# thiagopbueno/tf-mpc

Hardware: AMD Instinct MI355X
Metric: iLQR iterations/sec (batch x horizon) at n=16,m=8,T=50 (higher is better)
Workload: dtype f32

## Files before the change

tf-mpc_amd/csrc/lqr_mfma16x8.hip:

```cpp
#include <hip/hip_runtime.h>

#include <cstdlib>
#include <cstring>
#include <type_traits>

#include "lqr_kernels.h"
#include "options.h"
#include "mfma_bf16x3.h"
#include "wave_ldlt8.h"
#include "wave_ldlt8_pair.h"
#include "wave_ops.h"

namespace tfmpc {

namespace {

constexpr int N = 16, M = 8, D = 24;
using f32x4 = bf3::f32x4;

__device__ __forceinline__ f32x4 mfma(float a, float b, f32x4 c)
{
    return __builtin_amdgcn_mfma_f32_16x16x4f32(a, b, c, 0, 0, 0);
}

__device__ __forceinline__ float readlane(float v, int lane)
{
    return __builtin_bit_cast(float, __builtin_amdgcn_readlane(__builtin_bit_cast(int, v), lane));
}

using namespace bf3;

constexpr int kMs = 0;
constexpr int kKs = 256;
constexpr int kVt = 512;
constexpr int kVtLd = 20;
constexpr int kSweepFloats = kVt + 16 * kVtLd;
constexpr int kZs = 0;
constexpr int kZld = 26;
#ifndef TFMPC_LQR_TC
#define TFMPC_LQR_TC 52
#endif
constexpr int kTC = TFMPC_LQR_TC;
constexpr int kRolloutFloats = kZs + (kTC + 1) * kZld + 6;
constexpr int kLdsFloats = kSweepFloats > kRolloutFloats ? kSweepFloats : kRolloutFloats;
static_assert(kLdsFloats % 4 == 0, "slices are 16-byte aligned (pair_src, the 16-byte accesses of the sweep)");
#ifndef TFMPC_LQR_RING
#define TFMPC_LQR_RING 4
#endif
constexpr int kRing = TFMPC_LQR_RING;
static_assert(kTC % kRing == 0, "a chunk must hold whole turns of the gain ring");

template <int CTRL>
__device__ __forceinline__ float dpp(float v)
{
    return __builtin_bit_cast(float, __builtin_amdgcn_update_dpp(0, __builtin_bit_cast(int, v), CTRL, 0xF, 0xF, false));
}
constexpr int kDppXor1 = 0xB1;
constexpr int kDppXor2 = 0x4E;
constexpr int kDppHalfMirror = 0x141;

#define TFMPC_GLOBAL __attribute__((address_space(1)))
using gbytes = TFMPC_GLOBAL char *;
__device__ __forceinline__ gbytes uniform_base(const float *p)
{
    gbytes g = (gbytes)p;
    asm("" : "+s"(g));
    return g;
}
__device__ __forceinline__ unsigned here(unsigned &off)
{
    asm volatile("" : "+v"(off));
    return off;
}
template <class V>
__device__ __forceinline__ V gload(gbytes base, unsigned &off) { return *reinterpret_cast<const TFMPC_GLOBAL V *>(base + here(off)); }
template <class V>
__device__ __forceinline__ void gstore(gbytes base, unsigned &off, V v) { *reinterpret_cast<TFMPC_GLOBAL V *>(base + here(off)) = v; }
__device__ __forceinline__ int pinned(int v)
{
    asm("" : "+v"(v));
    return v;
}
typedef float f32x4_lds __attribute__((ext_vector_type(4), aligned(8)));
typedef float f32x4_any __attribute__((ext_vector_type(4), aligned(4)));

#ifdef TFMPC_LQR_EU
#define TFMPC_LQR_WAVES(EU_) TFMPC_LQR_EU
#else
#define TFMPC_LQR_WAVES(EU_) (EU_)
#endif
#define TFMPC_LQR_OCCUPANCY __attribute__((amdgpu_waves_per_eu(TFMPC_LQR_WAVES(EU), TFMPC_LQR_WAVES(EU))))
__device__ __forceinline__ void block_lds_sync()
{
    __builtin_amdgcn_fence(__ATOMIC_RELEASE, "workgroup", "local");
    __builtin_amdgcn_s_barrier();
    __builtin_amdgcn_fence(__ATOMIC_ACQUIRE, "workgroup", "local");
}
template <bool BACKWARD, bool FORWARD, bool VALUE, bool EXACT, bool BF3, bool OUT16 = false, int EU = 4, bool PAIR = false>
__global__ __launch_bounds__(PAIR ? 2 * kWave : kWave) TFMPC_LQR_OCCUPANCY void lqr_mfma16x8_kernel(LqrArgs a)
{
    static_assert(!PAIR || (BACKWARD && !VALUE && !OUT16), "the paired elimination serves the sweeps without value outputs");
    __shared__ __attribute__((aligned(16))) float lds_all[(PAIR ? 2 : 1) * kLdsFloats];
    const int wave = PAIR ? __builtin_amdgcn_readfirstlane(threadIdx.x >> 6) : 0;
    float *const lds = lds_all + wave * kLdsFloats;
    const int b_own = PAIR ? 2 * (int)blockIdx.x + wave : (int)blockIdx.x;
    const bool live = !PAIR || b_own < a.B;
    const int b = live ? b_own : a.B - 1;
    const int lane = PAIR ? (int)(threadIdx.x & (kWave - 1)) : (int)threadIdx.x;
    const int i = lane & 15, q = lane >> 4;
    const int T = a.T;
    const int n = EXACT ? N : a.n, m = EXACT ? M : a.m, d = n + m;
    auto Fxx = [&](const float *Fg, int row, int xi) { return (row < n && xi < n) ? Fg[row * d + xi] : 0.0f; };
    auto Fxu = [&](const float *Fg, int row, int ui) { return (row < n && ui < m) ? Fg[row * d + n + ui] : 0.0f; };
    auto zmap = [&](int zi) { return zi < N ? (zi < n ? zi : -1) : (zi - N < m ? n + zi - N : -1); };
    auto Czz = [&](const float *Cg, int zr, int zc) {
        const int r = zmap(zr), c_ = zmap(zc);
        return (r >= 0 && c_ >= 0) ? Cg[r * d + c_] : 0.0f;
    };
    auto cz = [&](const float *cg, int zr) { const int r = zmap(zr); return r >= 0 ? cg[r] : 0.0f; };
    const float *Fg = a.F + (size_t)b * a.sF;
    const float *fg = a.f + (size_t)b * a.sf;
    const float *Cg = a.C + (size_t)b * a.sC;
    const float *cg = a.c + (size_t)b * a.sc;
    float *Kg = a.K + (size_t)b * a.sK;
    float *kg = a.k + (size_t)b * a.sk;
    int status = 0;

    if (BACKWARD) {
        float Fb0[4], Fb1[4];
        f32x4 Cd00, Cd11;
        f32x4 Cd01t;
        f32x4 vterm;
#pragma unroll
        for (int r = 0; r < 4; ++r) {
            const int k = 4 * q + r;
            const int ku = N + k;
            if (EXACT) {
                Fb0[r] = Fg[k * D + i];
                Fb1[r] = (i < M) ? Fg[k * D + N + i] : ((i == M) ? fg[k] : 0.0f);
                Cd00[r] = Cg[k * D + i];
                Cd01t[r] = (k < M) ? Cg[(N + k) * D + i] : ((k == M) ? cg[i] : 0.0f);
                vterm[r] = (i == M) ? cg[k] : 0.0f;
                Cd11[r] = (ku < D) ? ((i < M) ? Cg[ku * D + N + i] : ((i == M) ? cg[ku] : 0.0f)) : 0.0f;
            } else {
                Fb0[r] = Fxx(Fg, k, i);
                Fb1[r] = (i < M) ? Fxu(Fg, k, i) : ((i == M && k < n) ? fg[k] : 0.0f);
                Cd00[r] = Czz(Cg, k, i);
                Cd01t[r] = (k < M) ? Czz(Cg, N + k, i) : ((k == M) ? cz(cg, i) : 0.0f);
                vterm[r] = (i == M) ? cz(cg, k) : 0.0f;
                float c11 = 0.0f;
                if (ku < D) {
                    if (i < M) c11 = (k >= m && i == k) ? 1.0f : Czz(Cg, ku, N + i);
                    else if (i == M) c11 = cz(cg, ku);
                }
                Cd11[r] = c11;
            }
        }
        ConstFrag Fc0{}, Fc1{};
        if (BF3) {
            Fc0 = const_frag(f32x4{Fb0[0], Fb0[1], Fb0[2], Fb0[3]});
            Fc1 = const_frag(f32x4{Fb1[0], Fb1[1], Fb1[2], Fb1[3]});
        }
        f32x4 Vd = Cd00, vd = vterm;
        float cst = 0.0f;
        int min_pivot_bits = 0x3f800000;
        int min_pivot_rows = 0x3f800000;
        const int pj = lane & 15, prow = (lane >> 4) & 1;
        const int pcol = pj >= 8 ? pj - 8 + 8 * prow : ((prow && pj == 0) ? N + M : N + pj);
        const int pair_src = PAIR ? 4 * pinned(((lane >> 5) * kLdsFloats + kMs + pcol * 8) / 4) : 0;
        const int pair_d0 = (lane >> 5) * kLdsFloats + kMs + N * 8;
        constexpr int kZero = kMs + 25 * 8;
        if (lane < kKs - kZero) lds[kZero + lane] = 0.0f;
        constexpr int kQx = kMs + 28 * 8;
        const int t01_src = (i == M) ? kQx + 4 * q : kZero;
        const int g1_src = (i == M) ? kKs + (N + M) * 8 + q : kZero + q;
        const int g0_src = pinned(kKs + i * 8 + q);
        const int vt_dst = pinned(kVt + 4 * q * kVtLd + i);
        unsigned offK = 8u * lane, offk = 4u * lane;
        __syncthreads();

        auto sweep_step = [&](const int t, auto LAST) __attribute__((always_inline)) {
            f32x4 W0 = {0.f, 0.f, 0.f, 0.f}, W1 = vd;
            if (BF3) {
                const VarFrag Vf = var_frag_block(Vd);
                W0 = mm_var_const(Vf, Fc0, W0);
                W1 = mm_var_const(Vf, Fc1, W1);
            } else {
#pragma unroll
                for (int r = 0; r < 4; ++r) {
                    W0 = mfma(Vd[r], Fb0[r], W0);
                    W1 = mfma(Vd[r], Fb1[r], W1);
                }
            }
            float fw = 0.0f, fv = 0.0f;
            if (VALUE) {
                float pw = 0.0f, pv = 0.0f;
#pragma unroll
                for (int r = 0; r < 4; ++r) {
                    pw = fmaf(Fb1[r], W1[r], pw);
                    pv = fmaf(Fb1[r], vd[r], pv);
                }
                fw = wave_sum(i == M ? pw : 0.0f);
                fv = wave_sum(i == M ? pv : 0.0f);
            }
            f32x4 T00 = Cd00, T01t = Cd01t, T11 = Cd11;
            if (BF3) {
                const VarFrag W0f = var_frag_block(W0), W1f = var_frag_block(W1);
                T00 = mm_const_var(Fc0, W0f, T00);
                T01t = mm_var_const(W1f, Fc0, T01t);
                T11 = mm_const_var(Fc1, W1f, T11);
            } else {
#pragma unroll
                for (int r = 0; r < 4; ++r) {
                    T00 = mfma(Fb0[r], W0[r], T00);
                    T01t = mfma(W1[r], Fb0[r], T01t);
                    T11 = mfma(Fb1[r], W1[r], T11);
                }
            }
            if (q < 2) {
                *reinterpret_cast<f32x4 *>(&lds[kMs + i * 8 + 4 * q]) = T01t;
                if (i <= M) *reinterpret_cast<f32x4 *>(&lds[kMs + (N + i) * 8 + 4 * q]) = T11;
            } else if (q == 2) {
                lds[kQx + i] = T01t[0];
            }
            float quk = 0.0f;
            if constexpr (PAIR) {
                block_lds_sync();
                if (wave == (t & 1)) {
                    f32x2 P2[4];
                    const f32x4 lo = *reinterpret_cast<const f32x4 *>(&lds_all[pair_src]);
                    const f32x4 hi = *reinterpret_cast<const f32x4 *>(&lds_all[pair_src + 4]);
                    const float d0 = lds_all[pair_d0];
                    P2[0] = f32x2{lo[0], lo[1]}; P2[1] = f32x2{lo[2], lo[3]};
                    P2[2] = f32x2{hi[0], hi[1]}; P2[3] = f32x2{hi[2], hi[3]};
                    float Pr[8];
                    ldlt8_pair_solve_neg(P2, Pr, d0, min_pivot_rows);
                    f32x4 klo, khi;
#pragma unroll
                    for (int r = 0; r < 4; ++r) { klo[r] = Pr[r]; khi[r] = Pr[4 + r]; }
                    *reinterpret_cast<f32x4 *>(&lds_all[pair_src + (kKs - kMs)]) = klo;
                    *reinterpret_cast<f32x4 *>(&lds_all[pair_src + (kKs - kMs) + 4]) = khi;
                }
                block_lds_sync();
            } else {
                lds_sync();
                f32x2 M2[4];
                {
                    const int c = lane & 31;
                    const f32x4 lo = *reinterpret_cast<const f32x4 *>(&lds[kMs + c * 8]);
                    const f32x4 hi = *reinterpret_cast<const f32x4 *>(&lds[kMs + c * 8 + 4]);
                    M2[0] = f32x2{lo[0], lo[1]}; M2[1] = f32x2{lo[2], lo[3]};
                    M2[2] = f32x2{hi[0], hi[1]}; M2[3] = f32x2{hi[2], hi[3]};
                }
                float qu_saved[8];
                if (VALUE) {
#pragma unroll
                    for (int p = 0; p < 8; ++p) qu_saved[p] = readlane(M2[p >> 1][p & 1], 24);
                }
                float Mr[8];
                ldlt8_solve_neg(M2, Mr, min_pivot_bits);
                if (VALUE) {
#pragma unroll
                    for (int p = 0; p < 8; ++p) quk = fmaf(readlane(Mr[p], 24), qu_saved[p], quk);
                }
                if (lane < 32) {
                    f32x4 lo, hi;
#pragma unroll
                    for (int r = 0; r < 4; ++r) { lo[r] = Mr[r]; hi[r] = Mr[4 + r]; }
                    *reinterpret_cast<f32x4 *>(&lds[kKs + lane * 8]) = lo;
                    *reinterpret_cast<f32x4 *>(&lds[kKs + lane * 8 + 4]) = hi;
                }
                lds_sync();
            }
            if constexpr (!decltype(LAST)::value) {
                f32x4 vacc = *reinterpret_cast<const f32x4 *>(&lds[t01_src]);
#pragma unroll
                for (int s2 = 0; s2 < 2; ++s2) {
                    const float ax = lds[kMs + i * 8 + 4 * s2 + q];
                    const float g0 = lds[g0_src + 4 * s2];
                    const float g1 = lds[g1_src + 4 * s2];
                    T00 = mfma(ax, g0, T00);
                    vacc = mfma(ax, g1, vacc);
                }
                {
                    const float *vt = &lds[kVt];
#pragma unroll
                    for (int r = 0; r < 4; ++r) lds[vt_dst + r * kVtLd] = T00[r];
                    lds_sync();
                    const f32x4 Tt = *reinterpret_cast<const f32x4 *>(&vt[i * kVtLd + 4 * q]);
#pragma unroll
                    for (int r = 0; r < 4; ++r) Vd[r] = 0.5f * (T00[r] + Tt[r]);
                }
                vd = vacc;
            }
            if (live) {
                const int ka = lane >> 3, jc = lane & 7;
                float2 kv;
                kv.x = lds[kKs + (2 * jc) * 8 + ka];
                kv.y = lds[kKs + (2 * jc + 1) * 8 + ka];
                if (EXACT) {
                    gstore(uniform_base(Kg + (size_t)t * (M * N)), offK, f32x2{kv.x, kv.y});
                    if (lane < M) gstore(uniform_base(kg + (size_t)t * M), offk, lds[kKs + 24 * 8 + lane]);
                } else {
                    if (ka < m && 2 * jc < n) Kg[(size_t)t * m * n + ka * n + 2 * jc] = kv.x;
                    if (ka < m && 2 * jc + 1 < n) Kg[(size_t)t * m * n + ka * n + 2 * jc + 1] = kv.y;
                    if (lane < m) kg[(size_t)t * m + lane] = lds[kKs + 24 * 8 + lane];
                }
                if (OUT16 && a.K16) {
                    uint16_t *Ko = a.K16 + ((size_t)b * T + t) * (m * n);
                    if (ka < m && 2 * jc < n) Ko[ka * n + 2 * jc] = lqr_to_bf16(kv.x);
                    if (ka < m && 2 * jc + 1 < n) Ko[ka * n + 2 * jc + 1] = lqr_to_bf16(kv.y);
                }
                if (OUT16 && a.k16 && lane < m) a.k16[((size_t)b * T + t) * m + lane] = lqr_to_bf16(lds[kKs + 24 * 8 + lane]);
            }
            if (VALUE) {
                cst += 0.5f * quk + 0.5f * (fw + fv);
                if (a.V) {
                    float *Vo = a.V + ((size_t)b * T + t) * (n * n);
#pragma unroll
                    for (int r = 0; r < 4; ++r)
                        if (EXACT || (4 * q + r < n && i < n)) Vo[(4 * q + r) * n + i] = Vd[r];
                }
                if (a.v && i == M) {
                    float *vo = a.v + ((size_t)b * T + t) * n;
#pragma unroll
                    for (int r = 0; r < 4; ++r)
                        if (EXACT || 4 * q + r < n) vo[4 * q + r] = vd[r];
                }
                if (a.cst && lane == 0) a.cst[(size_t)b * T + t] = cst;
                if (OUT16 && a.V16) {
                    uint16_t *Vo = a.V16 + ((size_t)b * T + t) * (n * n);
#pragma unroll
                    for (int r = 0; r < 4; ++r)
                        if (EXACT || (4 * q + r < n && i < n)) Vo[(4 * q + r) * n + i] = lqr_to_bf16(Vd[r]);
                }
                if (OUT16 && a.v16 && i == M) {
                    uint16_t *vo = a.v16 + ((size_t)b * T + t) * n;
#pragma unroll
                    for (int r = 0; r < 4; ++r)
                        if (EXACT || 4 * q + r < n) vo[4 * q + r] = lqr_to_bf16(vd[r]);
                }
                if (OUT16 && a.cst16 && lane == 0) a.cst16[(size_t)b * T + t] = lqr_to_bf16(cst);
            }
            lds_sync();
        };
        constexpr int kPeeled = VALUE ? 0 : 1;
        for (int t = T - 1; t >= kPeeled; --t) sweep_step(t, std::false_type{});
        if (kPeeled && T > 0) sweep_step(0, std::true_type{});
        if constexpr (PAIR) {
            constexpr int kMinPv = kKs + 25 * 8;
            if ((lane & 31) == 0) lds[kMinPv + (lane >> 5)] = __builtin_bit_cast(float, min_pivot_rows);
            block_lds_sync();
            const int p0 = __builtin_bit_cast(int, lds_all[kMinPv + wave]), p1 = __builtin_bit_cast(int, lds_all[kLdsFloats + kMinPv + wave]);
            min_pivot_bits = __builtin_amdgcn_readfirstlane(p0 < p1 ? p0 : p1);
        }
        if (min_pivot_bits <= 0) status |= (min_pivot_bits == 0) ? TFMPC_ST_SINGULAR : TFMPC_ST_NOT_PD;
        if (VALUE && !(cst == cst)) status |= TFMPC_ST_NAN;
    }

    const int lane_rollout = (BACKWARD && FORWARD) ? pinned((int)__builtin_amdgcn_mbcnt_hi(~0u, __builtin_amdgcn_mbcnt_lo(~0u, 0u))) : lane;
    if (FORWARD) {
        const int lane = lane_rollout, i = lane & 15, q = lane >> 4;
        const int fi = lane >> 2, fc = lane & 3;
        const int ka = lane >> 3, jc = lane & 7;
        float Fr[6];
        if (EXACT) {
            const float2 *p = reinterpret_cast<const float2 *>(Fg + fi * D + 6 * fc);
#pragma unroll
            for (int j = 0; j < 3; ++j) { const float2 v = p[j]; Fr[2 * j] = v.x; Fr[2 * j + 1] = v.y; }
        } else {
#pragma unroll
            for (int j = 0; j < 6; ++j) {
                const int zc = 6 * fc + j;
                Fr[j] = zc < N ? Fxx(Fg, fi, zc) : Fxu(Fg, fi, zc - N);
            }
        }
        const float f_part = (fc == 0 && (EXACT || fi < n)) ? fg[fi] : 0.0f;
        float Ca0[6], Ca1[6];
        f32x4 cq0, cq1;
#pragma unroll
        for (int s2 = 0; s2 < 6; ++s2) {
            if (EXACT) {
                Ca0[s2] = Cg[i * D + 4 * s2 + q];
                Ca1[s2] = (i < M) ? Cg[(N + i) * D + 4 * s2 + q] : 0.0f;
            } else {
                Ca0[s2] = Czz(Cg, i, 4 * s2 + q);
                Ca1[s2] = (i < M) ? Czz(Cg, N + i, 4 * s2 + q) : 0.0f;
            }
        }
#pragma unroll
        for (int r = 0; r < 4; ++r) {
            cq0[r] = EXACT ? cg[4 * q + r] : cz(cg, 4 * q + r);
            cq1[r] = (q < 2) ? (EXACT ? cg[N + 4 * q + r] : cz(cg, N + 4 * q + r)) : 0.0f;
        }
        float *xs = a.states + (size_t)b * (T + 1) * n;
        float *us = a.actions + (size_t)b * T * m;
        float *cs = a.costs + (size_t)b * (T + 1);
        float *zs = &lds[kZs];
        __syncthreads();
        if (lane < N) {
            const float x = (EXACT || lane < n) ? a.x0[(size_t)b * n + lane] : 0.0f;
            zs[lane] = x;
            if (live && (EXACT || lane < n)) xs[lane] = x;
        }
        unsigned offK = 8u * lane, offk = 4u * ka;
        auto load_gain = [&](int t, float2 &Kv, float &kv) {
            if (EXACT) {
                const f32x2 K2 = gload<f32x2>(uniform_base(Kg + (size_t)t * (M * N)), offK);
                Kv = float2{K2[0], K2[1]};
                kv = gload<float>(uniform_base(kg + (size_t)t * M), offk);
            } else {
                const bool row = ka < m;
                Kv.x = (row && 2 * jc < n) ? Kg[(size_t)t * m * n + ka * n + 2 * jc] : 0.0f;
                Kv.y = (row && 2 * jc + 1 < n) ? Kg[(size_t)t * m * n + ka * n + 2 * jc + 1] : 0.0f;
                kv = row ? kg[(size_t)t * m + ka] : 0.0f;
            }
        };
        float2 KR[kRing];
        float kR[kRing];
#pragma unroll
        for (int d = 0; d < kRing; ++d) {
            KR[d] = float2{0.f, 0.f};
            kR[d] = 0.0f;
            if (T > 0) load_gain(d < T ? d : T - 1, KR[d], kR[d]);
        }
        __syncthreads();

        auto chunk_costs = [&](int rows, float *out) {
            float part = 0.0f;
            for (int nt = 0; nt * 16 < rows; ++nt) {
                const int row = (16 * nt + i < rows) ? 16 * nt + i : rows - 1;
                const float *zrow = zs + row * kZld;
                f32x4 D0 = {0.f, 0.f, 0.f, 0.f}, D1 = {0.f, 0.f, 0.f, 0.f};
#pragma unroll
                for (int s2 = 0; s2 < 6; ++s2) {
                    const float bz = zrow[4 * s2 + q];
                    D0 = mfma(Ca0[s2], bz, D0);
                    D1 = mfma(Ca1[s2], bz, D1);
                }
                part = 0.0f;
#pragma unroll
                for (int r = 0; r < 4; ++r) {
                    part = fmaf(zrow[4 * q + r], fmaf(0.5f, D0[r], cq0[r]), part);
                    if (q < 2) part = fmaf(zrow[N + 4 * q + r], fmaf(0.5f, D1[r], cq1[r]), part);
                }
                part += __shfl_xor(part, 16, kWave);
                part += __shfl_xor(part, 32, kWave);
                if (live && q == 0 && 16 * nt + i < rows) {
                    unsigned offc = 4u * lane;
                    gstore(uniform_base(out + 16 * nt), offc, part);
                }
            }
            return part;
        };

        auto rollout_step = [&](const int tt, const int t, float2 &KRd, float &kRd, auto REFILL) __attribute__((always_inline)) {
            float *zt = zs + tt * kZld;
            const float2 Kc = KRd;
            const float kc = kRd;
            const float2 xv = *reinterpret_cast<const float2 *>(&zt[2 * jc]);
            float u = fmaf(Kc.x, xv.x, Kc.y * xv.y);
            u += dpp<kDppXor1>(u);
            u += dpp<kDppXor2>(u);
            u += dpp<kDppHalfMirror>(u);
            u += kc;
            if constexpr (decltype(REFILL)::value) load_gain(t + kRing < T ? t + kRing : T - 1, KRd, kRd);
            zt[N + ka] = u;
            lds_sync();
            float xn = f_part;
            const float2 *zp = reinterpret_cast<const float2 *>(&zt[6 * fc]);
#pragma unroll
            for (int j = 0; j < 3; ++j) {
                const float2 z2 = zp[j];
                xn = fmaf(Fr[2 * j], z2.x, xn);
                xn = fmaf(Fr[2 * j + 1], z2.y, xn);
            }
            xn += dpp<kDppXor1>(xn);
            xn += dpp<kDppXor2>(xn);
            zt[kZld + fi] = xn;
            lds_sync();
        };

        const int xrow = lane >> 2, urow = lane >> 1;
        const float *xsrc = zs + (1 + xrow) * kZld + 4 * (lane & 3);
        const float *usrc = zs + urow * kZld + N + 4 * (lane & 1);
        unsigned off16 = 16u * lane;
        auto rows_left = [](int v) { asm("" : "+s"(v)); return v; };

        for (int t0 = 0; t0 == 0 || t0 < T; t0 += kTC) {
            const bool last = T - t0 <= kTC;
            const int tc = last ? T - t0 : kTC;
            int tb = 0;
            for (; tb + kRing <= tc; tb += kRing) {
#pragma unroll
                for (int d = 0; d < kRing; ++d) rollout_step(tb + d, t0 + tb + d, KR[d], kR[d], std::true_type{});
            }
#pragma unroll
            for (int d = 0; d < kRing - 1; ++d)
                if (tb + d < tc) rollout_step(tb + d, t0 + tb + d, KR[d], kR[d], std::false_type{});
            if (last) {
                if (lane < M) zs[tc * kZld + N + lane] = __builtin_bit_cast(float, pinned(0));
                lds_sync();
            }
            const float tile_costs = chunk_costs(last ? tc + 1 : tc, cs + t0);
            if (last) {
                const float fcost = readlane(tile_costs, tc & 15);
                if (!(fcost == fcost)) status |= TFMPC_ST_NAN;
            }
            if (!live) {
            } else if (EXACT) {
                const gbytes xdst = uniform_base(xs + (size_t)(t0 + 1) * N), udst = uniform_base(us + (size_t)t0 * M);
#pragma unroll
                for (int r0 = 0; r0 < kTC; r0 += kWave / 4) {
                    const int left = rows_left(tc - r0);
                    if (left <= 0) break;
                    if (xrow < left)
                        gstore<f32x4_any>(xdst + r0 * (N * 4), off16, *reinterpret_cast<const f32x4_lds *>(xsrc + r0 * kZld));
                }
#pragma unroll
                for (int r0 = 0; r0 < kTC; r0 += kWave / 2) {
                    const int left = rows_left(tc - r0);
                    if (left <= 0) break;
                    if (urow < left)
                        gstore<f32x4_any>(udst + r0 * (M * 4), off16, *reinterpret_cast<const f32x4_lds *>(usrc + r0 * kZld));
                }
            } else {
                for (int idx = lane; idx < tc * n; idx += kWave)
                    xs[(size_t)(t0 + 1) * n + idx] = zs[(1 + idx / n) * kZld + idx % n];
                for (int idx = lane; idx < tc * m; idx += kWave)
                    us[(size_t)t0 * m + idx] = zs[(idx / m) * kZld + N + idx % m];
            }
            if (!last) {
                lds_sync();
                if (lane < N) zs[lane] = zs[kTC * kZld + lane];
                lds_sync();
            }
        }
    }

    if (live && a.status && lane_rollout == 0) a.status[b] = status;
}

bool use_bf16x3()
{
    return !option_is(kOptLqrMfma, "f32");
}

int pick_eu()
{
    const int forced = option_int(kOptLqrWaves, 0);
    return forced == 4 || forced == 6 ? forced : 5;
}

template <bool BW, bool FW, bool VAL, bool O16, int EU>
int launch_eu(const LqrArgs &a, hipStream_t stream)
{
    const bool exact = a.n == N && a.m == M;
    const bool bf3 = BW && use_bf16x3();
    constexpr bool P = BW && !VAL && !O16;
    const dim3 grid(P ? (a.B + 1) / 2 : a.B), block(P ? 2 * kWave : kWave);
    if (exact && bf3) hipLaunchKernelGGL((lqr_mfma16x8_kernel<BW, FW, VAL, true, true, O16, EU, P>), grid, block, 0, stream, a);
    else if (exact) hipLaunchKernelGGL((lqr_mfma16x8_kernel<BW, FW, VAL, true, false, O16, EU, P>), grid, block, 0, stream, a);
    else if (bf3) hipLaunchKernelGGL((lqr_mfma16x8_kernel<BW, FW, VAL, false, true, O16, EU, P>), grid, block, 0, stream, a);
    else hipLaunchKernelGGL((lqr_mfma16x8_kernel<BW, FW, VAL, false, false, O16, EU, P>), grid, block, 0, stream, a);
    return hipGetLastError() == hipSuccess ? TFMPC_OK : TFMPC_ERR_LAUNCH;
}

template <bool BW, bool FW, bool VAL, bool O16 = false>
int launch(const LqrArgs &a, hipStream_t stream)
{
    if constexpr (!VAL) {
        const int eu = pick_eu();
        if constexpr (BW && !O16) {
            if (eu == 6) return launch_eu<BW, FW, VAL, O16, 6>(a, stream);
        }
        if (eu >= 5) return launch_eu<BW, FW, VAL, O16, 5>(a, stream);
    }
    return launch_eu<BW, FW, VAL, O16, 4>(a, stream);
}

}

bool lqr_mfma_supported(int n, int m) { return n >= 1 && m >= 1 && n <= N && m <= M && n + m > 6; }

int lqr_mfma_launch(const LqrArgs &a, bool backward, bool forward, hipStream_t stream)
{
    if (a.K16 || a.k16 || a.V16 || a.v16 || a.cst16) {
        if (backward && forward) return launch<true, true, true, true>(a, stream);
        if (backward) return launch<true, false, true, true>(a, stream);
    }
    const bool value = a.V || a.v || a.cst;
    if (backward && forward) return value ? launch<true, true, true>(a, stream) : launch<true, true, false>(a, stream);
    if (backward) return value ? launch<true, false, true>(a, stream) : launch<true, false, false>(a, stream);
    return launch<false, true, false>(a, stream);
}

}
```

tf-mpc_amd/csrc/wave_ldlt8_pair.h:

```cpp
#pragma once

#include <hip/hip_runtime.h>

#include "wave_ldlt8.h"

namespace tfmpc {

#define TFMPC_BC(L) " row_newbcast:" #L " row_mask:0xf bank_mask:0xf\n\t"
#define TFMPC_PIVOT(P) "v_rcp_f32_dpp %[x" #P "], -%[m" #P "]" TFMPC_BC(P) \
                       "v_min_i32_dpp %[mp], %[m" #P "], %[mp]" TFMPC_BC(P) \
                       "v_mul_f32 %[x" #P "], %[m" #P "], %[x" #P "]\n\t"
#define TFMPC_FWD(P, S) "v_fmac_f32_dpp %[m" #S "], %[x" #P "], %[m" #P "]" TFMPC_BC(S)
#define TFMPC_BWD(P, O, S) "v_fmac_f32_dpp %[x" #P "], %[" #O "], %[x" #S "]" TFMPC_BC(S)
#define TFMPC_COPY(O, P) "v_mov_b32 %[" #O "], %[x" #P "]\n\t"

__device__ __forceinline__ void ldlt8_pair_solve_neg(const f32x2 (&M2)[4], float (&X)[8], float d0, int &min_pivot_bits)
{
    float M[8];
#pragma unroll
    for (int r = 0; r < 8; ++r) M[r] = M2[r >> 1][r & 1];
    asm("v_rcp_f32 %[x0], -%[d0]\n\t"
        "v_min_i32 %[mp], %[d0], %[mp]\n\t"
        "v_mul_f32 %[x0], %[m0], %[x0]\n\t"
        "s_nop 1\n\t"
        TFMPC_FWD(0, 1) TFMPC_FWD(0, 2) TFMPC_FWD(0, 3) TFMPC_FWD(0, 4) TFMPC_FWD(0, 5) TFMPC_FWD(0, 6) TFMPC_FWD(0, 7)
        TFMPC_PIVOT(1) "s_nop 1\n\t"
        TFMPC_FWD(1, 2) TFMPC_FWD(1, 3) TFMPC_FWD(1, 4) TFMPC_FWD(1, 5) TFMPC_FWD(1, 6) TFMPC_FWD(1, 7)
        TFMPC_PIVOT(2) "s_nop 1\n\t"
        TFMPC_FWD(2, 3) TFMPC_FWD(2, 4) TFMPC_FWD(2, 5) TFMPC_FWD(2, 6) TFMPC_FWD(2, 7)
        TFMPC_PIVOT(3) "s_nop 1\n\t"
        TFMPC_FWD(3, 4) TFMPC_FWD(3, 5) TFMPC_FWD(3, 6) TFMPC_FWD(3, 7)
        TFMPC_PIVOT(4) "s_nop 1\n\t"
        TFMPC_FWD(4, 5) TFMPC_FWD(4, 6) TFMPC_FWD(4, 7)
        TFMPC_PIVOT(5) "s_nop 1\n\t"
        TFMPC_FWD(5, 6) TFMPC_FWD(5, 7)
        "s_nop 0\n\t"
        TFMPC_PIVOT(6) "s_nop 1\n\t"
        TFMPC_FWD(6, 7)
        TFMPC_COPY(m0, 5) TFMPC_COPY(m1, 4)
        TFMPC_PIVOT(7)
        "v_fmac_f32_dpp %[x6], %[x6], %[x7]" TFMPC_BC(7)
        TFMPC_BWD(5, m0, 7) TFMPC_BWD(5, m0, 6)
        TFMPC_COPY(m0, 3)
        TFMPC_BWD(4, m1, 7) TFMPC_BWD(4, m1, 6) TFMPC_BWD(4, m1, 5)
        TFMPC_COPY(m1, 2)
        TFMPC_BWD(3, m0, 7) TFMPC_BWD(3, m0, 6) TFMPC_BWD(3, m0, 5) TFMPC_BWD(3, m0, 4)
        TFMPC_COPY(m0, 1)
        TFMPC_BWD(2, m1, 7) TFMPC_BWD(2, m1, 6) TFMPC_BWD(2, m1, 5) TFMPC_BWD(2, m1, 4) TFMPC_BWD(2, m1, 3)
        TFMPC_COPY(m1, 0)
        TFMPC_BWD(1, m0, 7) TFMPC_BWD(1, m0, 6) TFMPC_BWD(1, m0, 5) TFMPC_BWD(1, m0, 4) TFMPC_BWD(1, m0, 3) TFMPC_BWD(1, m0, 2)
        TFMPC_BWD(0, m1, 7) TFMPC_BWD(0, m1, 6) TFMPC_BWD(0, m1, 5) TFMPC_BWD(0, m1, 4) TFMPC_BWD(0, m1, 3) TFMPC_BWD(0, m1, 2) TFMPC_BWD(0, m1, 1)
        : [x0] "=&v"(X[0]), [x1] "=&v"(X[1]), [x2] "=&v"(X[2]), [x3] "=&v"(X[3]), [x4] "=&v"(X[4]), [x5] "=&v"(X[5]), [x6] "=&v"(X[6]),
          [x7] "=&v"(X[7]), [m0] "+v"(M[0]), [m1] "+v"(M[1]), [m2] "+v"(M[2]), [m3] "+v"(M[3]), [m4] "+v"(M[4]), [m5] "+v"(M[5]),
          [m6] "+v"(M[6]), [m7] "+v"(M[7]), [mp] "+v"(min_pivot_bits)
        : [d0] "v"(d0));
}
#undef TFMPC_COPY
#undef TFMPC_BWD
#undef TFMPC_FWD
#undef TFMPC_PIVOT
#undef TFMPC_BC

}
```

Baseline: 44.10 million.

## Fold value-vector update into the LDLT solve, dropping the g1 MFMA pass

After: 44.92 million (median of 6 runs). +1.9%, better.

```diff
diff --git a/tf-mpc_amd/csrc/lqr_mfma16x8.hip b/tf-mpc_amd/csrc/lqr_mfma16x8.hip
--- a/tf-mpc_amd/csrc/lqr_mfma16x8.hip
+++ b/tf-mpc_amd/csrc/lqr_mfma16x8.hip
@@ -60,6 +60,7 @@
 constexpr int kDppHalfMirror = 0x141;
 
 #define TFMPC_GLOBAL __attribute__((address_space(1)))
+#define TFMPC_LDS __attribute__((address_space(3)))
 using gbytes = TFMPC_GLOBAL char *;
 __device__ __forceinline__ gbytes uniform_base(const float *p)
 {
@@ -166,14 +167,15 @@
         int min_pivot_bits = 0x3f800000;
         int min_pivot_rows = 0x3f800000;
         const int pj = lane & 15, prow = (lane >> 4) & 1;
-        const int pcol = pj >= 8 ? pj - 8 + 8 * prow : ((prow && pj == 0) ? N + M : N + pj);
+        const int pcol = pj >= 8 ? pj - 8 + 8 * prow : (pj == 0 ? N + M : N + pj);
         const int pair_src = PAIR ? 4 * pinned(((lane >> 5) * kLdsFloats + kMs + pcol * 8) / 4) : 0;
         const int pair_d0 = (lane >> 5) * kLdsFloats + kMs + N * 8;
         constexpr int kZero = kMs + 25 * 8;
         if (lane < kKs - kZero) lds[kZero + lane] = 0.0f;
         constexpr int kQx = kMs + 28 * 8;
+        constexpr int kPark = kMs + 30 * 8;
+        const int pair_qx = (lane >> 5) * kLdsFloats + (pj >= 8 ? kQx + pj - 8 + 8 * prow : kPark + pj + 8 * prow);
         const int t01_src = (i == M) ? kQx + 4 * q : kZero;
-        const int g1_src = (i == M) ? kKs + (N + M) * 8 + q : kZero + q;
         const int g0_src = pinned(kKs + i * 8 + q);
         const int vt_dst = pinned(kVt + 4 * q * kVtLd + i);
         unsigned offK = 8u * lane, offk = 4u * lane;
@@ -231,10 +233,15 @@
                     const f32x4 lo = *reinterpret_cast<const f32x4 *>(&lds_all[pair_src]);
                     const f32x4 hi = *reinterpret_cast<const f32x4 *>(&lds_all[pair_src + 4]);
                     const float d0 = lds_all[pair_d0];
+                    const f32x4 qlo = *(const volatile TFMPC_LDS f32x4 *)&lds_all[pair_src];
+                    const f32x4 qhi = *(const volatile TFMPC_LDS f32x4 *)&lds_all[pair_src + 4];
+                    float vnext = lds_all[pair_qx];
                     P2[0] = f32x2{lo[0], lo[1]}; P2[1] = f32x2{lo[2], lo[3]};
                     P2[2] = f32x2{hi[0], hi[1]}; P2[3] = f32x2{hi[2], hi[3]};
+                    const float Qc[8] = {qlo[0], qlo[1], qlo[2], qlo[3], qhi[0], qhi[1], qhi[2], qhi[3]};
                     float Pr[8];
-                    ldlt8_pair_solve_neg(P2, Pr, d0, min_pivot_rows);
+                    ldlt8_pair_solve_neg(P2, Pr, d0, min_pivot_rows, Qc, vnext);
+                    lds_all[pair_qx] = vnext;
                     f32x4 klo, khi;
 #pragma unroll
                     for (int r = 0; r < 4; ++r) { klo[r] = Pr[r]; khi[r] = Pr[4 + r]; }
@@ -245,13 +252,17 @@
             } else {
                 lds_sync();
                 f32x2 M2[4];
+                float Qc[8];
                 {
                     const int c = lane & 31;
                     const f32x4 lo = *reinterpret_cast<const f32x4 *>(&lds[kMs + c * 8]);
                     const f32x4 hi = *reinterpret_cast<const f32x4 *>(&lds[kMs + c * 8 + 4]);
                     M2[0] = f32x2{lo[0], lo[1]}; M2[1] = f32x2{lo[2], lo[3]};
                     M2[2] = f32x2{hi[0], hi[1]}; M2[3] = f32x2{hi[2], hi[3]};
-                }
+#pragma unroll
+                    for (int r = 0; r < 4; ++r) { Qc[r] = lo[r]; Qc[4 + r] = hi[r]; }
+                }
+                float vnext = lds[kQx + (lane & 15)];
                 float qu_saved[8];
                 if (VALUE) {
 #pragma unroll
@@ -259,9 +270,17 @@
                 }
                 float Mr[8];
                 ldlt8_solve_neg(M2, Mr, min_pivot_bits);
+                float kb[8];
+#pragma unroll
+                for (int p = 0; p < 8; ++p) kb[p] = readlane(Mr[p], 24);
                 if (VALUE) {
 #pragma unroll
-                    for (int p = 0; p < 8; ++p) quk = fmaf(readlane(Mr[p], 24), qu_saved[p], quk);
+                    for (int p = 0; p < 8; ++p) quk = fmaf(kb[p], qu_saved[p], quk);
+                }
+                if constexpr (!decltype(LAST)::value) {
+#pragma unroll
+                    for (int p = 0; p < 8; ++p) vnext = fmaf(kb[p], Qc[p], vnext);
+                    if (lane < N) lds[kQx + lane] = vnext;
                 }
                 if (lane < 32) {
                     f32x4 lo, hi;
@@ -273,14 +292,12 @@
                 lds_sync();
             }
             if constexpr (!decltype(LAST)::value) {
-                f32x4 vacc = *reinterpret_cast<const f32x4 *>(&lds[t01_src]);
+                const f32x4 vacc = *reinterpret_cast<const f32x4 *>(&lds[t01_src]);
 #pragma unroll
                 for (int s2 = 0; s2 < 2; ++s2) {
                     const float ax = lds[kMs + i * 8 + 4 * s2 + q];
                     const float g0 = lds[g0_src + 4 * s2];
-                    const float g1 = lds[g1_src + 4 * s2];
                     T00 = mfma(ax, g0, T00);
-                    vacc = mfma(ax, g1, vacc);
                 }
                 {
                     const float *vt = &lds[kVt];
diff --git a/tf-mpc_amd/csrc/wave_ldlt8_pair.h b/tf-mpc_amd/csrc/wave_ldlt8_pair.h
--- a/tf-mpc_amd/csrc/wave_ldlt8_pair.h
+++ b/tf-mpc_amd/csrc/wave_ldlt8_pair.h
@@ -13,8 +13,10 @@
 #define TFMPC_FWD(P, S) "v_fmac_f32_dpp %[m" #S "], %[x" #P "], %[m" #P "]" TFMPC_BC(S)
 #define TFMPC_BWD(P, O, S) "v_fmac_f32_dpp %[x" #P "], %[" #O "], %[x" #S "]" TFMPC_BC(S)
 #define TFMPC_COPY(O, P) "v_mov_b32 %[" #O "], %[x" #P "]\n\t"
+#define TFMPC_VAL(A) "v_fmac_f32_dpp %[acc], %[x" #A "], %[q" #A "]" TFMPC_BC(0)
 
-__device__ __forceinline__ void ldlt8_pair_solve_neg(const f32x2 (&M2)[4], float (&X)[8], float d0, int &min_pivot_bits)
+__device__ __forceinline__ void ldlt8_pair_solve_neg(const f32x2 (&M2)[4], float (&X)[8], float d0, int &min_pivot_bits, const float (&Q)[8],
+                                                     float &acc)
 {
     float M[8];
 #pragma unroll
@@ -50,11 +52,15 @@
         TFMPC_COPY(m1, 0)
         TFMPC_BWD(1, m0, 7) TFMPC_BWD(1, m0, 6) TFMPC_BWD(1, m0, 5) TFMPC_BWD(1, m0, 4) TFMPC_BWD(1, m0, 3) TFMPC_BWD(1, m0, 2)
         TFMPC_BWD(0, m1, 7) TFMPC_BWD(0, m1, 6) TFMPC_BWD(0, m1, 5) TFMPC_BWD(0, m1, 4) TFMPC_BWD(0, m1, 3) TFMPC_BWD(0, m1, 2) TFMPC_BWD(0, m1, 1)
+        "s_nop 1\n\t"
+        TFMPC_VAL(0) TFMPC_VAL(1) TFMPC_VAL(2) TFMPC_VAL(3) TFMPC_VAL(4) TFMPC_VAL(5) TFMPC_VAL(6) TFMPC_VAL(7)
         : [x0] "=&v"(X[0]), [x1] "=&v"(X[1]), [x2] "=&v"(X[2]), [x3] "=&v"(X[3]), [x4] "=&v"(X[4]), [x5] "=&v"(X[5]), [x6] "=&v"(X[6]),
           [x7] "=&v"(X[7]), [m0] "+v"(M[0]), [m1] "+v"(M[1]), [m2] "+v"(M[2]), [m3] "+v"(M[3]), [m4] "+v"(M[4]), [m5] "+v"(M[5]),
-          [m6] "+v"(M[6]), [m7] "+v"(M[7]), [mp] "+v"(min_pivot_bits)
-        : [d0] "v"(d0));
+          [m6] "+v"(M[6]), [m7] "+v"(M[7]), [mp] "+v"(min_pivot_bits), [acc] "+v"(acc)
+        : [d0] "v"(d0), [q0] "v"(Q[0]), [q1] "v"(Q[1]), [q2] "v"(Q[2]), [q3] "v"(Q[3]), [q4] "v"(Q[4]), [q5] "v"(Q[5]), [q6] "v"(Q[6]),
+          [q7] "v"(Q[7]));
 }
+#undef TFMPC_VAL
 #undef TFMPC_COPY
 #undef TFMPC_BWD
 #undef TFMPC_FWD
```
